# lmxyy/sige

Hardware: AMD Instinct MI355X
Metric: DDPM-256 U-Net sparse (SIGE) forwards/s (higher is better)
Workload: dtype f32; 1 GPU; DDPM 256x256 church U-Net (ch128, mult 1-1-2-2-4-4, 113.7M params, random init), 1.2% square edit, one edited image per GPU, hipGraph replay, NHWC activations, in-place scatter ...; batch_per_gpu=1, resolution=256, parallelism=dp1

## Files before the change

### include/sige_hip.h

```cpp
#ifndef SIGE_HIP_H
#define SIGE_HIP_H

#include <stddef.h>
#include <stdint.h>

#ifdef __cplusplus
extern "C" {
#endif

#define SIGE_HIP_VERSION 310

enum {
    SIGE_HIP_OK = 0,
    SIGE_HIP_EINVAL = -1,
    SIGE_HIP_EUNSUPPORTED = -2,
    SIGE_HIP_ELAUNCH = -3,
    SIGE_HIP_ENODEVICE = -4
};

enum { SIGE_HIP_ACT_IDENTITY = 0, SIGE_HIP_ACT_SWISH = 1,
       SIGE_HIP_ACT_RELU = 2, SIGE_HIP_ACT_LEAKY = 3 , SIGE_HIP_ACT_TANH = 4 };

enum {
    SIGE_HIP_TUNE_CONV_TILE_MT = 0,
// ... 77 lines not shown
                            uint8_t *out, void *stream);
int sige_hip_mask_pyramid_levels(int H, int W, int min_h, int min_w, int *hs, int *ws, int capacity);
int sige_hip_mask_pyramid_u8(const uint8_t *mask, int H, int W, int min_h, int min_w,
                             int dilationH, int dilationW, float threshold, float eps,
                             float *scratch, size_t scratch_floats, uint8_t *out, void *stream);

int sige_hip_reduce_mask_capacity(int H, int W, int strideH, int strideW, int padH, int padW);
int sige_hip_reduce_mask_i32(const uint8_t *mask, int H, int W, int bH, int bW,
                             int strideH, int strideW, int padH, int padW,
                             int32_t *indices, int capacity, int32_t *count, void *stream);

int sige_hip_demand_tiles_capacity(int Hp, int Wp, int tileH, int tileW);
int sige_hip_demand_tiles_i32(const int32_t *indices, const int32_t *count, int capacity, int bH, int bW,
                              int inH, int inW, int upsample2x, int Hp, int Wp, int tileH, int tileW,
                              int padH, int padW, int depth, int32_t *lists, int32_t *counts, void *stream);

size_t sige_hip_block_conv_packed_size(int Cout, int Cin, int kH, int kW, int R, int S,
                                       int strideH, int strideW, int groups);
int sige_hip_block_conv_pack_f32(const float *w, int Cout, int Cin, int kH, int kW,
                                 float *packed, void *stream);
int sige_hip_block_conv_f32(const float *x, int T, int Cin, int R, int S,
                            const float *packed, const float *bias, int Cout, int kH, int kW,
                            int strideH, int strideW, float *out, void *stream);
int sige_hip_block_conv_direct_f32(const float *x, int T, int Cin, int R, int S,
                                   const float *w, const float *bias, int Cout, int kH, int kW,
                                   int strideH, int strideW, int dilationH, int dilationW, int groups,
                                   float *out, void *stream);
int sige_hip_spade_modulate_nhwc_f32(
        const float *x_full, const float *x_tiles, const int32_t *map_x, int Nx, int Rx, int Sx,
        const float *scale, int scaleB, int scaleC, const float *shift, int shiftB, int shiftC,
// ... 287 lines not shown
```

### sige_amd/csrc/mask_pipeline.hip

```cpp
#include "common.hpp"

namespace sige {

constexpr int kMPThreads = 1024;

__global__ void difference_mask_kernel(const float *__restrict__ a, const float *__restrict__ b, int C, long HW,
                                       long strideC, long stridePix, float eps, uint8_t *__restrict__ out) {
    for (long p = (long)blockIdx.x * blockDim.x + threadIdx.x; p < HW; p += (long)gridDim.x * blockDim.x) {
        bool any = false;
        for (int c = 0; c < C; ++c) {
            const long o = c * strideC + p * stridePix;
            any |= fabsf(a[o] - b[o]) > eps;
        }
        out[p] = any ? 1 : 0;
    }
}

__device__ __forceinline__ uint8_t dilated(const uint8_t *__restrict__ m, int W, int h, int w, int dH, int dW, int lo, int hi) {
    if (m[(size_t)h * W + w]) return 1;
    for (int i = 1; i <= dH; ++i) {
        if (h - i >= lo && m[(size_t)(h - i) * W + w]) return 1;
        if (h + i < hi && m[(size_t)(h + i) * W + w]) return 1;
    }
    for (int i = 1; i <= dW; ++i) {
// ... 67 lines not shown
            auto at = [&](int y, int x) -> float {
                const size_t q = (size_t)y * w + x;
                return cur ? cur[q] : (mask[q] ? 1.0f : 0.0f);
            };
            nxt[p] = hy * (hx * at(y0, x0) + lx * at(y0, x1)) + ly * (hx * at(y1, x0) + lx * at(y1, x1));
        }
        __syncthreads();
        cur = nxt;
        nxt = (nxt == level_a) ? level_b : level_a;
        h = h2; w = w2;
    }
}

constexpr int kDTThreads = 1024, kDTMaxPix = 16384, kDTMaxCells = 4096;

__global__ __launch_bounds__(kDTThreads) void demand_tiles_kernel(
        const int32_t *__restrict__ idx, const int32_t *__restrict__ count, int capacity, int bH, int bW, int inH, int inW, int up,
        int Hp, int Wp, int oH, int oW, int padH, int padW, int depth, int32_t *__restrict__ lists, int32_t *__restrict__ counts) {
    __shared__ uint8_t s_map[2][kDTMaxPix];
    __shared__ uint8_t s_flag[kDTMaxCells];
    const int tid = threadIdx.x;
    const int npix = Hp * Wp, gh = (Hp + oH - 1) / oH, gw = (Wp + oW - 1) / oW, ncell = gh * gw;
    for (int p = tid; p < npix; p += kDTThreads) s_map[0][p] = 0;
    __syncthreads();
    int n = *count;
    n = n < 0 ? 0 : (n > capacity ? capacity : n);
    const int bpix = bH * bW;
    for (long i = tid; i < (long)n * bpix; i += kDTThreads) {
        const int t = (int)(i / bpix), r = (int)(i % bpix);
        const int y = idx[2 * t] + r / bW, x = idx[2 * t + 1] + r % bW;
        if (y < 0 || y >= inH || x < 0 || x >= inW) continue;
        const int py = y >> up, px = x >> up;
        if (py < Hp && px < Wp) s_map[0][py * Wp + px] = 1;
    }
    __syncthreads();
    int cur = 0;
    for (int k = 0; k < depth; ++k) {
        const uint8_t *m = s_map[cur];
        for (int c = tid; c < ncell; c += kDTThreads) {
            const int y0 = (c / gw) * oH, x0 = (c % gw) * oW;
            const int y1 = y0 + oH < Hp ? y0 + oH : Hp, x1 = x0 + oW < Wp ? x0 + oW : Wp;
            uint8_t any = 0;
            for (int y = y0; y < y1; ++y)
                for (int x = x0; x < x1; ++x) any |= m[y * Wp + x];
            s_flag[c] = any;
        }
        __syncthreads();
        int32_t *main_list = lists + (size_t)k * ncell * 2, *flat_list = lists + ((size_t)depth + k) * ncell * 2;
        for (int c = tid; c < ncell; c += kDTThreads) {
            if (!s_flag[c] && c != ncell - 1) continue;
            int rank = 0;
            for (int j = 0; j < c; ++j) rank += s_flag[j];
            if (s_flag[c]) {
                const int y0 = (c / gw) * oH, x0 = (c % gw) * oW;
                main_list[2 * rank] = y0 - padH; main_list[2 * rank + 1] = x0 - padW;
                flat_list[2 * rank] = y0; flat_list[2 * rank + 1] = x0;
            }
            if (c == ncell - 1) counts[k] = rank + s_flag[c];
        }
        if (k + 1 < depth) {
            uint8_t *d = s_map[cur ^ 1];
            for (int p = tid; p < npix; p += kDTThreads) {
                const int y = p / Wp, x = p % Wp;
                uint8_t any = 0;
                for (int yy = (y > 0 ? y - 1 : 0); yy <= (y + 1 < Hp ? y + 1 : Hp - 1); ++yy)
                    for (int xx = (x > 0 ? x - 1 : 0); xx <= (x + 1 < Wp ? x + 1 : Wp - 1); ++xx) any |= m[yy * Wp + xx];
                d[p] = any;
            }
        }
        __syncthreads();
        cur ^= 1;
    }
}

}

using namespace sige;

extern "C" int sige_hip_demand_tiles_capacity(int Hp, int Wp, int tileH, int tileW) {
    if (Hp <= 0 || Wp <= 0 || tileH <= 0 || tileW <= 0) return SIGE_HIP_EINVAL;
    return ((Hp + tileH - 1) / tileH) * ((Wp + tileW - 1) / tileW);
}

extern "C" int sige_hip_demand_tiles_i32(const int32_t *indices, const int32_t *count, int capacity, int bH, int bW,
                                         int inH, int inW, int upsample2x, int Hp, int Wp, int tileH, int tileW,
                                         int padH, int padW, int depth, int32_t *lists, int32_t *counts, void *stream) {
    SIGE_PLAN_HOOK(sige_hip_demand_tiles_i32, indices, count, capacity, bH, bW, inH, inW, upsample2x, Hp, Wp, tileH, tileW, padH, padW, depth, lists, counts, stream);
    if (capacity < 0 || bH <= 0 || bW <= 0 || inH <= 0 || inW <= 0 || Hp <= 0 || Wp <= 0 || tileH <= 0 || tileW <= 0 ||
        padH < 0 || padW < 0 || depth <= 0)
        return SIGE_HIP_EINVAL;
    if (!count || !lists || !counts || (capacity > 0 && !indices)) return SIGE_HIP_EINVAL;
    const int up = upsample2x ? 1 : 0;
    if (inH != (Hp << up) || inW != (Wp << up)) return SIGE_HIP_EINVAL;
    if (stacked_shift(Hp) != 0) return SIGE_HIP_EUNSUPPORTED;
    if ((long)Hp * Wp > kDTMaxPix || sige_hip_demand_tiles_capacity(Hp, Wp, tileH, tileW) > kDTMaxCells) return SIGE_HIP_EUNSUPPORTED;
    demand_tiles_kernel<<<1, kDTThreads, 0, as_stream(stream)>>>(indices, count, capacity, bH, bW, inH, inW, up, Hp, Wp, tileH, tileW,
                                                                padH, padW, depth, lists, counts);
    return launch_status();
}

extern "C" int sige_hip_difference_mask_u8(const float *a, const float *b, int C, int H, int W,
                                           int64_t strideC, int64_t strideH, int64_t strideW, float eps,
                                           uint8_t *out, void *stream) {
    SIGE_PLAN_HOOK(sige_hip_difference_mask_u8, a, b, C, H, W, strideC, strideH, strideW, eps, out, stream);
    if (C <= 0 || H <= 0 || W <= 0) return SIGE_HIP_EINVAL;
    if (!a || !b || !out) return SIGE_HIP_EINVAL;
    if (strideH != (int64_t)W * strideW) return SIGE_HIP_EUNSUPPORTED;
    const long HW = (long)H * W;
    const int blocks = (int)((HW + 255) / 256 < 2048 ? (HW + 255) / 256 : 2048);
    difference_mask_kernel<<<blocks, 256, 0, as_stream(stream)>>>(a, b, C, HW, strideC, strideW, eps, out);
    return launch_status();
}
// ... 48 lines not shown
```

### sige_amd/hip.py

```python
import ctypes
import os
import threading
from typing import Optional, Tuple

import torch

_PKG = os.path.dirname(os.path.abspath(__file__))
LIB_PATH = os.environ.get("SIGE_HIP_LIB", os.path.join(_PKG, "lib", "libsige_hip.so"))

ACT = {"identity": 0, "swish": 1}
ACT_EXT = {"identity": 0, "relu": 2, "leaky": 3, "tanh": 4}

_c_int, _c_vp, _c_sz = ctypes.c_int, ctypes.c_void_p, ctypes.c_size_t
_lib = None

_BC = [_c_vp, _c_int, _c_int, _c_int, _c_int]

_SIGNATURES = {
    "sige_hip_version": (_c_int, []),
    "sige_hip_error_string": (ctypes.c_char_p, [_c_int]),
    "sige_hip_device_arch": (ctypes.c_char_p, []),
    "sige_hip_launch_count": (ctypes.c_int64, []),
    "sige_hip_last_launch_device": (_c_int, []),
    "sige_hip_preload": (_c_int, []),
# ... 4 lines not shown
    "sige_hip_tile_table_i32": (_c_int, [_c_vp] + [_c_int] * 9 + [_c_vp, _c_vp]),
    "sige_hip_scatter_fused_f32": (_c_int, [_c_vp, _c_vp] + [_c_int] * 6 + [_c_vp, _c_int, _c_int, _c_int] + _BC + [_c_vp, _c_vp]),
    "sige_hip_scatter_with_block_residual_fused_f32": (
        _c_int, [_c_vp] * 4 + [_c_int] * 8 + [_c_vp, _c_int, _c_int, _c_int] * 2 + [_c_vp, _c_vp]),
    "sige_hip_scatter_map_i32": (_c_int, [_c_int] * 10 + [_c_vp, _c_int, _c_vp, _c_vp]),
    "sige_hip_scatter_gather_f32": (
        _c_int, [_c_vp, _c_vp] + [_c_int] * 8 + [_c_vp, _c_int, _c_vp] + _BC + _BC + [_c_int, _c_int, _c_vp, _c_vp]),
    "sige_hip_difference_mask_u8": (_c_int, [_c_vp, _c_vp] + [_c_int] * 3 + [ctypes.c_int64] * 3 + [ctypes.c_float, _c_vp, _c_vp]),
    "sige_hip_dilate_mask_u8": (_c_int, [_c_vp] + [_c_int] * 4 + [_c_vp, _c_vp]),
    "sige_hip_mask_pyramid_levels": (_c_int, [_c_int] * 4 + [_c_vp, _c_vp, _c_int]),
    "sige_hip_mask_pyramid_u8": (_c_int, [_c_vp] + [_c_int] * 6 + [ctypes.c_float] * 2 + [_c_vp, _c_sz, _c_vp, _c_vp]),
    "sige_hip_reduce_mask_capacity": (_c_int, [_c_int] * 6),
    "sige_hip_reduce_mask_i32": (_c_int, [_c_vp] + [_c_int] * 8 + [_c_vp, _c_int, _c_vp, _c_vp]),
    "sige_hip_demand_tiles_capacity": (_c_int, [_c_int] * 4),
    "sige_hip_demand_tiles_i32": (_c_int, [_c_vp, _c_vp] + [_c_int] * 13 + [_c_vp, _c_vp, _c_vp]),
    "sige_hip_block_conv_packed_size": (_c_sz, [_c_int] * 9),
    "sige_hip_block_conv_packed_size_f16c": (_c_sz, [_c_int] * 9),
    "sige_hip_block_conv_pack_f16c": (_c_int, [_c_vp] + [_c_int] * 4 + [_c_vp, _c_vp]),
    "sige_hip_block_conv_pack_f32": (_c_int, [_c_vp] + [_c_int] * 4 + [_c_vp, _c_vp]),
    "sige_hip_block_conv_f32": (_c_int, [_c_vp] + [_c_int] * 4 + [_c_vp, _c_vp] + [_c_int] * 5 + [_c_vp, _c_vp]),
    "sige_hip_gather_conv_f32": (
        _c_int, [_c_vp] + [_c_int] * 6 + [_c_vp, _c_int] + _BC + _BC + [_c_int, _c_vp, _c_vp] + [_c_int] * 5 + [_c_vp, _c_vp]),
    "sige_hip_scatter_gather_conv_f32": (
        _c_int, [_c_vp, _c_vp] + [_c_int] * 8 + [_c_vp, _c_int, _c_vp] + _BC + _BC + [_c_int, _c_vp, _c_vp]
        + [_c_int] * 5 + [_c_vp, _c_vp]),
    "sige_hip_gather_conv_nchw_f32": (
        _c_int, [_c_vp, _c_vp] + [_c_int] * 7 + [_c_vp, _c_int] + [_c_vp, _c_int, _c_int] * 2 + [_c_int, _c_vp, _c_vp]
        + [_c_int] * 7 + [_c_vp, _c_int, _c_int, _c_vp, _c_vp]),
    "sige_hip_group_norm_affine_workspace": (_c_sz, [_c_int] * 5),
    "sige_hip_group_norm_affine_f32": (_c_int, [_c_vp] + [_c_int] * 5 + [ctypes.c_float] + [_c_vp] * 6),
# ... 505 lines not shown
                                          _stream(m)), "reduce_mask")
    n = int(count[0].item())
    return buf[:n].clone()


class DemandTiles:

    def __init__(self, main, flat, cells: int):
        self.main, self.flat, self.cells = list(main), list(flat), int(cells)

    @property
    def counts(self):
        return [int(t.shape[0]) for t in self.main]


def reduce_mask_batch(requests, demands=None):
    if not requests:
        return [] if demands is None else ([], [])
    dev = requests[0][0].device
    n_req = len(requests)
    counts = torch.empty(n_req + sum(d[6] for d in demands or ()), dtype=torch.int32, device=dev)
    bufs = []
    for i, (mask, block, stride, padding) in enumerate(requests):
        if mask.dim() != 2 or not mask.is_cuda or mask.device != dev:
            raise RuntimeError("sige_amd.hip.reduce_mask_batch: expected 2-D masks on one GPU")
        m = mask if mask.dtype in (torch.bool, torch.uint8) else (mask != 0)
        m = m.contiguous()
        H, W = m.shape
        cap = lib().sige_hip_reduce_mask_capacity(H, W, stride[0], stride[1], padding[0], padding[1])
        buf = torch.empty((max(cap, 1), 2), dtype=torch.int32, device=dev)
        _check(lib().sige_hip_reduce_mask_i32(m.data_ptr(), H, W, block[0], block[1], stride[0], stride[1],
                                              padding[0], padding[1], buf.data_ptr(), cap,
                                              counts.data_ptr() + 4 * i, _stream(m)), "reduce_mask")
        bufs.append((buf, m, cap))
    dbufs, at = [], n_req
    for (i, in_res, up, prod_res, out_tile, pad, depth) in demands or ():
        buf, m, cap = bufs[i]
        block = requests[i][1]
        cells = lib().sige_hip_demand_tiles_capacity(prod_res[0], prod_res[1], out_tile[0], out_tile[1])
        if cells <= 0:
            raise RuntimeError("sige_amd.hip.reduce_mask_batch: bad demand-region geometry")
        lists = torch.empty((2, depth, cells, 2), dtype=torch.int32, device=dev)
        _check(lib().sige_hip_demand_tiles_i32(buf.data_ptr(), counts.data_ptr() + 4 * i, cap, block[0], block[1], in_res[0], in_res[1],
                                               int(bool(up)), prod_res[0], prod_res[1], out_tile[0], out_tile[1], pad[0], pad[1],
                                               depth, lists.data_ptr(), counts.data_ptr() + 4 * at, _stream(m)), "demand_tiles")
        dbufs.append((lists, at, depth, cells))
        at += depth
    rec = plan_recorder()
    if rec is not None:
        first = rec.new_slots(counts.numel())
        _check(lib().sige_hip_plan_record_readback(rec.handle, counts.data_ptr(), first, counts.numel()), "plan_record_readback")
        ns = counts.cpu().tolist()
        out = []
        for i, ((buf, m, _), n) in enumerate(zip(bufs, ns)):
            rec.bind_index_list(buf, first + i, n)
            rec.keep.extend((buf, m))
            out.append(buf[:n])
        dout = []
        for lists, at, depth, cells in dbufs:
            for g in range(2):
                for k in range(depth):
                    rec.bind_index_list(lists[g, k], first + at + k, ns[at + k])
            rec.keep.append(lists)
            dout.append(DemandTiles([lists[0, k, :ns[at + k]] for k in range(depth)],
                                    [lists[1, k, :ns[at + k]] for k in range(depth)], cells))
        rec.keep.append(counts)
        return out if demands is None else (out, dout)
    ns = counts.cpu().tolist()
    out = [buf[:n].clone() for (buf, _, _), n in zip(bufs, ns)]
    if demands is None:
        return out
    dout = [DemandTiles([lists[0, k, :ns[at + k]] for k in range(depth)], [lists[1, k, :ns[at + k]] for k in range(depth)], cells)
            for lists, at, depth, cells in dbufs]
    return out, dout


def difference_mask(tensor1: torch.Tensor, tensor2: torch.Tensor, eps: float) -> torch.Tensor:
    if tensor1.shape != tensor2.shape:
        raise RuntimeError("difference_mask: shapes differ")
    a, b = tensor1, tensor2
    if a.dim() == 4:
        assert a.shape[0] == 1
        a, b = a[0], b[0]
    if a.dim() == 2:
        a, b = a[None], b[None]
    if a.dim() != 3:
        raise NotImplementedError("Unknown mask dimension [%d]!!!" % tensor1.dim())
    if not (a.is_cuda and b.is_cuda and a.dtype == b.dtype == torch.float32):
        raise NotImplementedError("difference_mask: fp32 GPU tensors")
# ... 1358 lines not shown
```

### sige_amd/nn/base.py

```python
from typing import Dict, List, Optional, Tuple

import torch
from torch import nn
from torch.nn import functional as F

from .. import runtime as _runtime
from . import deferred

MODES = ("full", "sparse", "profile")


class _RuntimeTable(dict):

    def __init__(self, function_name: str):
        super().__init__()
        self.function_name = function_name

    def __missing__(self, device_type: str):
        fn = _runtime.resolve(device_type, self.function_name)
        if fn is not None:
            self[device_type] = fn
        return fn


# ... 198 lines not shown
        for m in self._sige_modules():
            if isinstance(m, Gather) and m.input_res is not None and not m.verbose:
                res = tuple(m.input_res)
                mask = masks.get(res)
                key = m.index_key(res)
                if mask is not None and mask.is_cuda and mask.dim() == 2 and key not in cache and key not in keys:
                    keys.append(key)
                    reqs.append((mask, m.block_size, m.block_stride, m.offset))
        self._demand_lists = {}
        demands = []
        for name, g, up, prod_res, depth in self._demand_requests(masks):
            key = g.index_key(tuple(g.input_res))
            if key in keys:
                demands.append((name, ("demand_tiles", *key[1:], int(up), *prod_res, *g.out_tile, *g.offset, depth),
                                (keys.index(key), tuple(g.input_res), up, tuple(prod_res), tuple(g.out_tile), tuple(g.offset), depth)))
        if reqs:
            from .. import hip

            lists, regions = hip.reduce_mask_batch(reqs, [d[2] for d in demands])
            for key, idx in zip(keys, lists):
                cache[key] = idx
            for (name, key, _), region in zip(demands, regions):
                cache[key] = region
                self._demand_lists[name] = region

    def _demand_requests(self, masks):
        return []

    def adopt_index_lists(self, view_of):
        for region in getattr(self, "_demand_lists", {}).values():
            for lists in (region.main, region.flat):
                for k, t in enumerate(lists):
                    v = view_of(t)
                    if v is not None:
                        lists[k] = v

    def set_mode(self, mode: str):
        self.mode = mode
        for module in self._sige_modules():
            module.set_mode(mode)

    def clear_cache(self):
        for module in self._sige_modules():
            module.clear_cache()

# ... 48 lines not shown
```

### sige_amd/nn/dense.py

```python
from typing import Optional, Tuple

import torch
from torch import nn
from torch.nn import functional as F

_GEOMETRY = {
    ((3, 3), (1, 1), (1, 1)): ((6, 6), (4, 4), (1, 1)),
    ((1, 1), (1, 1), (0, 0)): ((4, 4), (4, 4), (0, 0)),
    ((3, 3), (2, 2), (0, 0)): ((5, 5), (2, 2), (0, 0)),
}


def _tile_compute(compute: str) -> str:
    return compute if compute in ("f16", "f16x3") else "f32"


WIDE_MIN_FLOP = {3: 4.0e9, 1: 2.0e9}
WIDE_MIN_FLOP_X3 = {3: 4.0e9, 1: 2.0e9}
WIDE_MIN_FLOP_FULL_PASS = {3: 0.25e9, 1: 2.0e9}
WIDE_MIN_FLOP_F32 = {3: 1.0e30, 1: 1.0e30}
WIDE_MIN_FLOP_F32_STACKED = {3: 8.0e9, 1: 1.0e30}
FULL_PASS_F32_NATIVE = False
TILE_X3_MIN_FLOP = 2.0e9

# ... 144 lines not shown
            made = scatter.emulated_twins(out, twins)
    out._sige_twins = made
    return out


def demand_buffer(conv: nn.Conv2d, name, shape, device) -> torch.Tensor:
    bufs = conv.__dict__.setdefault("_sige_demand_bufs", {})
    buf = bufs.get(name)
    if buf is None or tuple(buf.shape) != tuple(shape) or buf.device != device:
        buf = torch.zeros(tuple(shape), dtype=torch.float32, device=device).contiguous(memory_format=torch.channels_last)
        bufs[name] = buf
    return buf


def _demand_twin_buffers(conv: nn.Conv2d, keys, shape, device):
    bufs = conv.__dict__.setdefault("_sige_demand_bufs", {})
    for name in [n for n in bufs if isinstance(n, tuple) and n[0] == "twin" and n[1] not in keys]:
        del bufs[name]
    return [demand_buffer(conv, ("twin", k), shape, device) for k in keys]


def _fused_conv2d(conv, x, scale, shift, activation_name, x2, residual, pad_bottom_right, out_affine, twins=None, made=None,
                  tiles=None, out_buf=None):
    if x.is_cuda and x.dtype == torch.float32 and fusable(conv):
        from .. import hip

        block, out_tile, offset = _GEOMETRY[(tuple(conv.kernel_size), tuple(conv.stride), tuple(conv.padding))]
        partial = (tiles is not None and out_buf is not None and not pad_bottom_right and conv.stride[0] == 1 and hip.is_cl(x)
                   and (x2 is None or (hip.is_cl(x2) and hip.cat_fusable(x.shape[0], x.shape[1], conv.kernel_size)))
                   and hip.cl_supported(x.shape[1], 0 if x2 is None else x2.shape[1], conv.out_channels))
        if partial:
            B, _, H, W = x.shape
# ... 120 lines not shown
```

### sige_amd/plan.py

```python
import ctypes
from typing import Callable, Dict, Optional

import torch

from . import hip
from .graphs import GraphPool
from .nn.base import SIGEModel
from .nn.gather import Gather

MASKS, FORWARD = 0, 1


class _Recorder:

    def __init__(self, plan: "LaunchPlan", section: int):
        self.plan = plan
        self.handle = plan.handle
        self.section = section
        self.keep = plan._keep
        self.idx_info = plan._idx_info

    def new_slots(self, n: int) -> int:
        first = hip.lib().sige_hip_plan_new_slots(self.handle, n)
        if first < 0:
# ... 67 lines not shown
            raise ValueError("LaunchPlan.record: `mask` must be a 2-D bool tensor on the GPU")
        self.build_masks, self.forward = build_masks, forward
        with torch.cuda.device(self.device):
            self.mask = mask.clone()
            self.model.set_mode("sparse")
            self.model.set_masks(build_masks(self.mask))
            eager = None
            for _ in range(max(1, warmup)):
                eager = forward()
            eager = eager.clone()
            with LaunchPlan._Recording(self, MASKS):
                self.model.set_masks(build_masks(self.mask))
                for m in self._scatter_modules():
                    m.plan_tables()
                    m.refresh_outputs(new_mask=True)
            torch.cuda.synchronize(self.device)
            self.pool = GraphPool(self.device)
            with LaunchPlan._Recording(self, FORWARD):
                self._record_graph, self.out = self.pool.capture(forward)
            if hip.lib().sige_hip_plan_calls(self.handle, FORWARD) <= 0:
                raise RuntimeError("LaunchPlan.record: the forward made no library call")
            self._read_counts()
            self._recorded_counts = list(self.counts)
            if not all(self.counts):
                raise RuntimeError("LaunchPlan.record: record under a mask with at least one active tile at every resolution (an empty "
                                   "index list hands the entry points a null pointer, which no later mask can be looked up under)")
            out = self.run()
            if check:
                torch.cuda.synchronize(self.device)
                err = float((out - eager).abs().max())
# ... 83 lines not shown
```

### sige_amd/utils.py

```python
from typing import Dict, Optional, Tuple, Union

import numpy as np
import torch
from torch.nn import functional as F

IntPair = Union[int, Tuple[int, int]]


def _pair(v: IntPair) -> Tuple[int, int]:
    return (v, v) if isinstance(v, int) else (int(v[0]), int(v[1]))


def reduce_mask(
    mask: torch.Tensor,
    block_size: Optional[IntPair],
    stride: Optional[IntPair],
    padding: Optional[IntPair],
    verbose: bool = False,
) -> Optional[torch.Tensor]:
    if block_size is None or stride is None or padding is None:
        return None
    block_size, stride, padding = _pair(block_size), _pair(stride), _pair(padding)
    if mask.is_cuda:
        from . import hip
# ... 121 lines not shown
    for k in range(depth):
        padded = torch.zeros((gh * oh, gw * ow), dtype=torch.bool)
        padded[:hp, :wp] = need
        cells = torch.nonzero(padded.reshape(gh, oh, gw, ow).any(dim=3).any(dim=1))
        origin = torch.stack((cells[:, 0] * oh, cells[:, 1] * ow), dim=1).to(torch.int32)
        flat.append(origin.contiguous())
        main.append((origin - torch.tensor([ph, pw], dtype=torch.int32)).contiguous())
        if k + 1 < depth:
            grown = need.clone()
            for dy in (-1, 0, 1):
                for dx in (-1, 0, 1):
                    src = need[max(-dy, 0):hp - max(dy, 0), max(-dx, 0):wp - max(dx, 0)]
                    grown[max(dy, 0):hp - max(-dy, 0), max(dx, 0):wp - max(-dx, 0)] |= src
            need = grown
    return main, flat
```

### sige_amd/workloads/ddpm_unet.py

```python
import math
from dataclasses import dataclass
from typing import Optional, Tuple

import torch
from torch import nn
from torch.nn import functional as F

from ..nn import Gather, Scatter, ScatterGather, ScatterWithBlockResidual, SIGEConv2d, SIGEModel, SIGEModule, paired_convs
from ..nn.deferred import lazy_cat
from ..nn.dense import demand_buffer, fast_full_pass, full_conv2d, fused_conv2d, group_norm_affine, input_conv2d


@dataclass
class DDPMConfig:
    ch: int = 128
    ch_mult: Tuple[int, ...] = (1, 1, 2, 2, 4, 4)
    num_res_blocks: int = 2
    attn_resolutions: Tuple[int, ...] = (16,)
    in_ch: int = 3
    out_ch: int = 3
    resolution: int = 256
    main_block: Optional[int] = 6
    shortcut_block: Optional[int] = 4
    sparse_threshold: int = 64
# ... 207 lines not shown

    def _pairing(self, t: torch.Tensor):
        return paired_convs(t, enabled=self.pair and self.cin != self.cout and self.mode == "sparse")

    def forward(self, x, temb: Optional[torch.Tensor], demand=None) -> torch.Tensor:
        pair = x if isinstance(x, (tuple, list)) else None
        if self.mode == "full":
            if pair and not self.plain and self._fast_full() and pair[0].is_cuda:
                return self._full(pair[0], temb, x2=pair[1])
            return self._full(torch.cat(pair, dim=1) if pair else x, temb)
        if self.mode in ("sparse", "profile"):
            if pair and not self.sparse_main and self.mode == "sparse":
                return self._sparse_dense(pair[0], pair[1], demand)
            if pair and self.mode == "sparse" and self.cin != self.cout:
                return self._sparse(lazy_cat(pair[0], pair[1]))
            return self._sparse(torch.cat(pair, dim=1) if pair else x)
        raise NotImplementedError("Unknown mode [%s]!!!" % self.mode)

    def _fast_full(self) -> bool:
        from ..nn import dense as _dense

        return _dense.fast_full_pass(self.conv1)

    def _shortcut(self, x, x2=None):
        if self.cin == self.cout:
            return x if x2 is None else torch.cat([x, x2], dim=1)
        if x2 is not None:
            if self.sparse_shortcut:
                self.shortcut_gather.note_full_input(x.shape[2:])
            return full_conv2d(self.nin_shortcut, x, x2=x2)
        if self.sparse_shortcut:
# ... 28 lines not shown
            s2, t2 = norm_affine(h + _as4(te), self.norm2, fast)
            t2 = t2 + te * s2
        self._drop_twin_links()
        self.affine[self.cache_id] = tuple(_as4(v).contiguous() for v in (s1, t1, s2, t2))
        if self.sparse_main and self.preactivate:
            self.scatter_gather.cache_activated(_as4(s2), _as4(t2))
        if self.sparse_main and self.sparse_shortcut:
            if fast and h.is_cuda:
                h = full_conv2d(self.conv2, h, _as4(s2), _as4(t2), "swish", residual=skip, stats=True)
                return self.scatter(h, skip, x_is_sum=True)
            h = full_conv2d(self.conv2, h, _as4(s2), _as4(t2), "swish")
            return self.scatter(h, skip)
        h = full_conv2d(self.conv2, h, _as4(s2), _as4(t2), "swish", residual=skip, stats=fast)
        return self.scatter(h) if self.sparse_main else h

    def _sparse(self, x):
        s1, t1, s2, t2 = self.affine[self.cache_id]
        if self.sparse_main and self.preactivate and self.mode == "sparse":
            parts = list(x.parts) if hasattr(x, "parts") else [x]
            first = parts[0]
            tw = self._twin_inputs(parts, s1, t1)
            with self._pairing(first):
                skip, join = (self._shortcut_async(lambda: self._shortcut(x), first) if self.cin != self.cout
                              else (x, lambda: None))
                if tw is not None:
                    xa = tw[0] if len(tw) == 1 else lazy_cat(tw[0], tw[1])
                    h = self.conv1(self.main_gather(xa, preactivated=True), out_affine=(s2, t2, "swish"))
                else:
                    h = self.conv1(self.main_gather(x, s1, t1), out_affine=(s2, t2, "swish"))
            tiles = self.scatter_gather(h, preactivated=True)
            join()
            return self._produced(self.scatter.forward_fused(self.conv2, tiles, skip))
        if not self.sparse_main:
            return self._sparse_dense(x, None)
        skip = self._shortcut(x)
        h = self.conv1(self.main_gather(x, s1, t1))
        if self.mode == "sparse":
            return self.scatter.forward_fused(self.conv2, self.scatter_gather(h, s2, t2), skip)
        return self.scatter(self.conv2(self.scatter_gather(h, s2, t2)), skip)

    def _demand_args(self, conv, demand, deeper: int, x) -> dict:
        if demand is None:
            return {}
        from .. import hip

        region, depth = demand
        lists = region.flat if tuple(conv.kernel_size) == (1, 1) else region.main
        tiles = lists[depth + deeper]
        if tiles.shape[0] == region.cells and hip.plan_recorder() is None:
            return {}
        shape = (x.shape[0], conv.out_channels, x.shape[2], x.shape[3])
        return dict(tiles=tiles, out=demand_buffer(conv, "out", shape, x.device))

    def _sparse_dense(self, x, x2, demand=None):
        s1, t1, s2, t2 = self.affine[self.cache_id]
        join = lambda: None
        if self.preactivate:
            tw = self._twin_inputs([x] if x2 is None else [x, x2], s1, t1)
            with self._pairing(x):
                if self.cin == self.cout:
                    skip = x if x2 is None else torch.cat([x, x2], dim=1)
                else:
                    skip, join = self._shortcut_async(lambda: fused_conv2d(self.nin_shortcut, x, x2=x2,
                                                                           **self._demand_args(self.nin_shortcut, demand, 0, x)), x)
                if tw is not None:
                    h = fused_conv2d(self.conv1, tw[0], None, None, "identity", x2=(tw[1] if len(tw) > 1 else None),
                                     out_affine=(s2, t2, "swish"), **self._demand_args(self.conv1, demand, 1, x))
# ... 394 lines not shown
        if not (self.DENSE_ON_DEMAND and self.mode == "sparse" and self.edit_batch == 1 and isinstance(h, torch.Tensor) and h.is_cuda):
            return None
        region = getattr(self, "_demand_lists", {}).get("up.%d" % lvl)
        if region is None or h.shape[0] != 1:
            return None
        from .. import hip

        convs = [c for b in stage.block for c in (b.conv1, b.conv2, getattr(b, "nin_shortcut", None)) if c is not None]
        if not hip.is_cl(h) or any(getattr(c, "compute_dtype", "f32") != "f32" for c in convs):
            return None
        g = stage.upsample.gather
        if not g.fuses_upsample(h) or tuple(g.input_res) != (2 * h.shape[2], 2 * h.shape[3]):
            return None
        return region

    def forward(self, x: torch.Tensor, t: torch.Tensor) -> torch.Tensor:
        assert x.shape[2] == x.shape[3] == self.resolution
        temb = self._temb(t)
        nxt = (lambda: temb.pop(0)) if temb is not None else (lambda: None)

        from ..nn import dense as _dense

        native_full = self.mode == "full" and x.is_cuda and not getattr(self.conv_in, "_plain_model", False) and (
            getattr(self.conv_out, "compute_dtype", "f32") != "f32" or _dense.FULL_PASS_F32_NATIVE)
        h0 = self._conv_in(x, native_full)
        if x.is_contiguous(memory_format=torch.channels_last) and not x.is_contiguous():
            h0 = h0.contiguous(memory_format=torch.channels_last)
        E = self.edit_batch
        if E > 1:
            if self.mode != "sparse" or x.shape[0] != E:
                raise RuntimeError("stacked edits: sparse mode, one input image per edit")
            from ..stacked import tall, untall

            h0 = tall(h0)
        hs = [h0]
        for lvl, stage in enumerate(self.down):
            for i, block in enumerate(stage.block):
                h = block(hs[-1], nxt())
                if len(stage.attn):
                    h = stage.attn[i](h)
                hs.append(h)
            if lvl != self.num_levels - 1:
                hs.append(stage.downsample(hs[-1]))

        h = self.mid.block_1(hs[-1], nxt())
        h = self.mid.attn_1(h)
        h = self.mid.block_2(h, nxt())

        for lvl in reversed(range(self.num_levels)):
            stage = self.up[lvl]
            region = self._stage_demand(lvl, stage, h)
            for i, block in enumerate(stage.block):
                if region is not None:
# ... 15 lines not shown
```

Before: 817.8 forward/s.

## Restrict dense down-stage convs to change regions grown from the sparse mask

Adds a change-tiles kernel that projects the downsample's active blocks to the next level and dilates them once per 3x3 conv, producing per-conv tile lists of cells whose output can differ from the cached original. Dense down stages without attention then run their convs only on those tiles, writing into persistent tagged output buffers. The buffers are first filled by a full-tile build pass keyed by a signature. This cuts work at dense down levels but adds state tracking, a cache-invalidation signature and an extra tile-list kernel, and it is only correct while the cached buffers stay valid.

```diff
diff --git a/include/sige_hip.h b/include/sige_hip.h
--- a/include/sige_hip.h
+++ b/include/sige_hip.h
@@ -115,6 +115,11 @@
 int sige_hip_demand_tiles_i32(const int32_t *indices, const int32_t *count, int capacity, int bH, int bW,
                               int inH, int inW, int upsample2x, int Hp, int Wp, int tileH, int tileW,
                               int padH, int padW, int depth, int32_t *lists, int32_t *counts, void *stream);
+
+int sige_hip_change_tiles_i32(const int32_t *indices, const int32_t *count, int capacity, int bH, int bW,
+                              int strideH, int strideW, int offsetH, int offsetW, int outH, int outW,
+                              int Hp, int Wp, int tileH, int tileW, int padH, int padW, int depth,
+                              int32_t *lists, int32_t *counts, void *stream);
 
 size_t sige_hip_block_conv_packed_size(int Cout, int Cin, int kH, int kW, int R, int S,
                                        int strideH, int strideW, int groups);
diff --git a/sige_amd/csrc/mask_pipeline.hip b/sige_amd/csrc/mask_pipeline.hip
--- a/sige_amd/csrc/mask_pipeline.hip
+++ b/sige_amd/csrc/mask_pipeline.hip
@@ -105,13 +105,51 @@
 
 constexpr int kDTThreads = 1024, kDTMaxPix = 16384, kDTMaxCells = 4096;
 
+__device__ __forceinline__ void dt_compact(const uint8_t *m, uint8_t *s_flag, int Hp, int Wp, int oH, int oW, int padH, int padW,
+                                           int32_t *__restrict__ main_list, int32_t *__restrict__ flat_list, int32_t *__restrict__ n_out) {
+    const int tid = threadIdx.x;
+    const int gh = (Hp + oH - 1) / oH, gw = (Wp + oW - 1) / oW, ncell = gh * gw;
+    for (int c = tid; c < ncell; c += kDTThreads) {
+        const int y0 = (c / gw) * oH, x0 = (c % gw) * oW;
+        const int y1 = y0 + oH < Hp ? y0 + oH : Hp, x1 = x0 + oW < Wp ? x0 + oW : Wp;
+        uint8_t any = 0;
+        for (int y = y0; y < y1; ++y)
+            for (int x = x0; x < x1; ++x) any |= m[y * Wp + x];
+        s_flag[c] = any;
+    }
+    __syncthreads();
+    for (int c = tid; c < ncell; c += kDTThreads) {
+        if (!s_flag[c] && c != ncell - 1) continue;
+        int rank = 0;
+        for (int j = 0; j < c; ++j) rank += s_flag[j];
+        if (s_flag[c]) {
+            const int y0 = (c / gw) * oH, x0 = (c % gw) * oW;
+            main_list[2 * rank] = y0 - padH; main_list[2 * rank + 1] = x0 - padW;
+            flat_list[2 * rank] = y0; flat_list[2 * rank + 1] = x0;
+        }
+        if (c == ncell - 1) *n_out = rank + s_flag[c];
+    }
+    __syncthreads();
+}
+
+__device__ __forceinline__ void dt_dilate(const uint8_t *m, uint8_t *d, int Hp, int Wp) {
+    for (int p = threadIdx.x; p < Hp * Wp; p += kDTThreads) {
+        const int y = p / Wp, x = p % Wp;
+        uint8_t any = 0;
+        for (int yy = (y > 0 ? y - 1 : 0); yy <= (y + 1 < Hp ? y + 1 : Hp - 1); ++yy)
+            for (int xx = (x > 0 ? x - 1 : 0); xx <= (x + 1 < Wp ? x + 1 : Wp - 1); ++xx) any |= m[yy * Wp + xx];
+        d[p] = any;
+    }
+    __syncthreads();
+}
+
 __global__ __launch_bounds__(kDTThreads) void demand_tiles_kernel(
         const int32_t *__restrict__ idx, const int32_t *__restrict__ count, int capacity, int bH, int bW, int inH, int inW, int up,
         int Hp, int Wp, int oH, int oW, int padH, int padW, int depth, int32_t *__restrict__ lists, int32_t *__restrict__ counts) {
     __shared__ uint8_t s_map[2][kDTMaxPix];
     __shared__ uint8_t s_flag[kDTMaxCells];
     const int tid = threadIdx.x;
-    const int npix = Hp * Wp, gh = (Hp + oH - 1) / oH, gw = (Wp + oW - 1) / oW, ncell = gh * gw;
+    const int npix = Hp * Wp, ncell = ((Hp + oH - 1) / oH) * ((Wp + oW - 1) / oW);
     for (int p = tid; p < npix; p += kDTThreads) s_map[0][p] = 0;
     __syncthreads();
     int n = *count;
@@ -127,40 +165,40 @@
     __syncthreads();
     int cur = 0;
     for (int k = 0; k < depth; ++k) {
-        const uint8_t *m = s_map[cur];
-        for (int c = tid; c < ncell; c += kDTThreads) {
-            const int y0 = (c / gw) * oH, x0 = (c % gw) * oW;
-            const int y1 = y0 + oH < Hp ? y0 + oH : Hp, x1 = x0 + oW < Wp ? x0 + oW : Wp;
-            uint8_t any = 0;
-            for (int y = y0; y < y1; ++y)
-                for (int x = x0; x < x1; ++x) any |= m[y * Wp + x];
-            s_flag[c] = any;
-        }
-        __syncthreads();
-        int32_t *main_list = lists + (size_t)k * ncell * 2, *flat_list = lists + ((size_t)depth + k) * ncell * 2;
-        for (int c = tid; c < ncell; c += kDTThreads) {
-            if (!s_flag[c] && c != ncell - 1) continue;
-            int rank = 0;
-            for (int j = 0; j < c; ++j) rank += s_flag[j];
-            if (s_flag[c]) {
-                const int y0 = (c / gw) * oH, x0 = (c % gw) * oW;
-                main_list[2 * rank] = y0 - padH; main_list[2 * rank + 1] = x0 - padW;
-                flat_list[2 * rank] = y0; flat_list[2 * rank + 1] = x0;
-            }
-            if (c == ncell - 1) counts[k] = rank + s_flag[c];
-        }
-        if (k + 1 < depth) {
-            uint8_t *d = s_map[cur ^ 1];
-            for (int p = tid; p < npix; p += kDTThreads) {
-                const int y = p / Wp, x = p % Wp;
-                uint8_t any = 0;
-                for (int yy = (y > 0 ? y - 1 : 0); yy <= (y + 1 < Hp ? y + 1 : Hp - 1); ++yy)
-                    for (int xx = (x > 0 ? x - 1 : 0); xx <= (x + 1 < Wp ? x + 1 : Wp - 1); ++xx) any |= m[yy * Wp + xx];
-                d[p] = any;
-            }
-        }
-        __syncthreads();
+        dt_compact(s_map[cur], s_flag, Hp, Wp, oH, oW, padH, padW, lists + (size_t)k * ncell * 2,
+                   lists + ((size_t)depth + k) * ncell * 2, counts + k);
+        if (k + 1 < depth) dt_dilate(s_map[cur], s_map[cur ^ 1], Hp, Wp);
         cur ^= 1;
+    }
+}
+
+__global__ __launch_bounds__(kDTThreads) void change_tiles_kernel(
+        const int32_t *__restrict__ idx, const int32_t *__restrict__ count, int capacity, int sH, int sW, int offH, int offW,
+        int tH, int tW, int Hp, int Wp, int oH, int oW, int padH, int padW, int depth, int32_t *__restrict__ lists,
+        int32_t *__restrict__ counts) {
+    __shared__ uint8_t s_map[2][kDTMaxPix];
+    __shared__ uint8_t s_flag[kDTMaxCells];
+    const int tid = threadIdx.x;
+    const int npix = Hp * Wp, ncell = ((Hp + oH - 1) / oH) * ((Wp + oW - 1) / oW);
+    for (int p = tid; p < npix; p += kDTThreads) s_map[0][p] = 0;
+    __syncthreads();
+    int n = *count;
+    n = n < 0 ? 0 : (n > capacity ? capacity : n);
+    const int tpix = tH * tW;
+    for (long i = tid; i < (long)n * tpix; i += kDTThreads) {
+        const int t = (int)(i / tpix), r = (int)(i % tpix);
+        const int ty = idx[2 * t] + offH, tx = idx[2 * t + 1] + offW;
+        if (ty < 0 || tx < 0) continue;
+        const int y = ty / sH + r / tW, x = tx / sW + r % tW;
+        if (y < Hp && x < Wp) s_map[0][y * Wp + x] = 1;
+    }
+    __syncthreads();
+    int cur = 0;
+    for (int k = 0; k < depth; ++k) {
+        dt_dilate(s_map[cur], s_map[cur ^ 1], Hp, Wp);
+        cur ^= 1;
+        dt_compact(s_map[cur], s_flag, Hp, Wp, oH, oW, padH, padW, lists + (size_t)k * ncell * 2,
+                   lists + ((size_t)depth + k) * ncell * 2, counts + k);
     }
 }
 
@@ -187,6 +225,23 @@
     if ((long)Hp * Wp > kDTMaxPix || sige_hip_demand_tiles_capacity(Hp, Wp, tileH, tileW) > kDTMaxCells) return SIGE_HIP_EUNSUPPORTED;
     demand_tiles_kernel<<<1, kDTThreads, 0, as_stream(stream)>>>(indices, count, capacity, bH, bW, inH, inW, up, Hp, Wp, tileH, tileW,
                                                                 padH, padW, depth, lists, counts);
+    return launch_status();
+}
+
+extern "C" int sige_hip_change_tiles_i32(const int32_t *indices, const int32_t *count, int capacity, int bH, int bW,
+                                         int strideH, int strideW, int offsetH, int offsetW, int outH, int outW,
+                                         int Hp, int Wp, int tileH, int tileW, int padH, int padW, int depth,
+                                         int32_t *lists, int32_t *counts, void *stream) {
+    SIGE_PLAN_HOOK(sige_hip_change_tiles_i32, indices, count, capacity, bH, bW, strideH, strideW, offsetH, offsetW, outH, outW, Hp, Wp, tileH, tileW, padH, padW, depth, lists, counts, stream);
+    if (capacity < 0 || bH <= 0 || bW <= 0 || strideH <= 0 || strideW <= 0 || offsetH < 0 || offsetW < 0 || outH <= 0 || outW <= 0 ||
+        Hp <= 0 || Wp <= 0 || tileH <= 0 || tileW <= 0 || padH < 0 || padW < 0 || depth <= 0)
+        return SIGE_HIP_EINVAL;
+    if (!count || !lists || !counts || (capacity > 0 && !indices)) return SIGE_HIP_EINVAL;
+    if ((long)(outH - 1) * strideH >= bH || (long)(outW - 1) * strideW >= bW) return SIGE_HIP_EINVAL;
+    if (stacked_shift(Hp) != 0) return SIGE_HIP_EUNSUPPORTED;
+    if ((long)Hp * Wp > kDTMaxPix || sige_hip_demand_tiles_capacity(Hp, Wp, tileH, tileW) > kDTMaxCells) return SIGE_HIP_EUNSUPPORTED;
+    change_tiles_kernel<<<1, kDTThreads, 0, as_stream(stream)>>>(indices, count, capacity, strideH, strideW, offsetH, offsetW, outH, outW,
+                                                                Hp, Wp, tileH, tileW, padH, padW, depth, lists, counts);
     return launch_status();
 }
 
diff --git a/sige_amd/hip.py b/sige_amd/hip.py
--- a/sige_amd/hip.py
+++ b/sige_amd/hip.py
@@ -42,6 +42,7 @@
     "sige_hip_reduce_mask_i32": (_c_int, [_c_vp] + [_c_int] * 8 + [_c_vp, _c_int, _c_vp, _c_vp]),
     "sige_hip_demand_tiles_capacity": (_c_int, [_c_int] * 4),
     "sige_hip_demand_tiles_i32": (_c_int, [_c_vp, _c_vp] + [_c_int] * 13 + [_c_vp, _c_vp, _c_vp]),
+    "sige_hip_change_tiles_i32": (_c_int, [_c_vp, _c_vp] + [_c_int] * 16 + [_c_vp, _c_vp, _c_vp]),
     "sige_hip_block_conv_packed_size": (_c_sz, [_c_int] * 9),
     "sige_hip_block_conv_packed_size_f16c": (_c_sz, [_c_int] * 9),
     "sige_hip_block_conv_pack_f16c": (_c_int, [_c_vp] + [_c_int] * 4 + [_c_vp, _c_vp]),
@@ -577,12 +578,17 @@
         return [int(t.shape[0]) for t in self.main]
 
 
-def reduce_mask_batch(requests, demands=None):
+class ChangeTiles(DemandTiles):
+    """Index lists of a dense stage's change regions (include/sige_hip.h: sige_hip_change_tiles_i32): `main[k-1]` / `flat[k-1]` =
+    the cells on which the output of the stage's k-th 3x3 conv can differ from the original's, in the 3x3 and the 1x1 geometry."""
+
+
+def reduce_mask_batch(requests, demands=None, changes=None):
     if not requests:
-        return [] if demands is None else ([], [])
+        return [] if demands is None else (([], []) if changes is None else ([], [], []))
     dev = requests[0][0].device
     n_req = len(requests)
-    counts = torch.empty(n_req + sum(d[6] for d in demands or ()), dtype=torch.int32, device=dev)
+    counts = torch.empty(n_req + sum(d[6] for d in demands or ()) + sum(c[7] for c in changes or ()), dtype=torch.int32, device=dev)
     bufs = []
     for i, (mask, block, stride, padding) in enumerate(requests):
         if mask.dim() != 2 or not mask.is_cuda or mask.device != dev:
@@ -607,7 +613,21 @@
         _check(lib().sige_hip_demand_tiles_i32(buf.data_ptr(), counts.data_ptr() + 4 * i, cap, block[0], block[1], in_res[0], in_res[1],
                                                int(bool(up)), prod_res[0], prod_res[1], out_tile[0], out_tile[1], pad[0], pad[1],
                                                depth, lists.data_ptr(), counts.data_ptr() + 4 * at, _stream(m)), "demand_tiles")
-        dbufs.append((lists, at, depth, cells))
+        dbufs.append((lists, at, depth, cells, DemandTiles))
+        at += depth
+    n_dem = len(dbufs)
+    for (i, stride, wrote, offset, prod_res, out_tile, pad, depth) in changes or ():
+        buf, m, cap = bufs[i]
+        block = requests[i][1]
+        cells = lib().sige_hip_demand_tiles_capacity(prod_res[0], prod_res[1], out_tile[0], out_tile[1])
+        if cells <= 0:
+            raise RuntimeError("sige_amd.hip.reduce_mask_batch: bad change-region geometry")
+        lists = torch.empty((2, depth, cells, 2), dtype=torch.int32, device=dev)
+        _check(lib().sige_hip_change_tiles_i32(buf.data_ptr(), counts.data_ptr() + 4 * i, cap, block[0], block[1], stride[0], stride[1],
+                                               offset[0], offset[1], wrote[0], wrote[1], prod_res[0], prod_res[1],
+                                               out_tile[0], out_tile[1], pad[0], pad[1], depth, lists.data_ptr(),
+                                               counts.data_ptr() + 4 * at, _stream(m)), "change_tiles")
+        dbufs.append((lists, at, depth, cells, ChangeTiles))
         at += depth
     rec = plan_recorder()
     if rec is not None:
@@ -620,22 +640,22 @@
             rec.keep.extend((buf, m))
             out.append(buf[:n])
         dout = []
-        for lists, at, depth, cells in dbufs:
+        for lists, at, depth, cells, kind in dbufs:
             for g in range(2):
                 for k in range(depth):
                     rec.bind_index_list(lists[g, k], first + at + k, ns[at + k])
             rec.keep.append(lists)
-            dout.append(DemandTiles([lists[0, k, :ns[at + k]] for k in range(depth)],
-                                    [lists[1, k, :ns[at + k]] for k in range(depth)], cells))
+            dout.append(kind([lists[0, k, :ns[at + k]] for k in range(depth)],
+                             [lists[1, k, :ns[at + k]] for k in range(depth)], cells))
         rec.keep.append(counts)
-        return out if demands is None else (out, dout)
-    ns = counts.cpu().tolist()
-    out = [buf[:n].clone() for (buf, _, _), n in zip(bufs, ns)]
-    if demands is None:
-        return out
-    dout = [DemandTiles([lists[0, k, :ns[at + k]] for k in range(depth)], [lists[1, k, :ns[at + k]] for k in range(depth)], cells)
-            for lists, at, depth, cells in dbufs]
-    return out, dout
+    else:
+        ns = counts.cpu().tolist()
+        out = [buf[:n].clone() for (buf, _, _), n in zip(bufs, ns)]
+        dout = [kind([lists[0, k, :ns[at + k]] for k in range(depth)], [lists[1, k, :ns[at + k]] for k in range(depth)], cells)
+                for lists, at, depth, cells, kind in dbufs]
+    if changes is not None:
+        return out, dout[:n_dem], dout[n_dem:]
+    return out if demands is None else (out, dout)
 
 
 def difference_mask(tensor1: torch.Tensor, tensor2: torch.Tensor, eps: float) -> torch.Tensor:
diff --git a/sige_amd/nn/base.py b/sige_amd/nn/base.py
--- a/sige_amd/nn/base.py
+++ b/sige_amd/nn/base.py
@@ -236,21 +236,34 @@
             if key in keys:
                 demands.append((name, ("demand_tiles", *key[1:], int(up), *prod_res, *g.out_tile, *g.offset, depth),
                                 (keys.index(key), tuple(g.input_res), up, tuple(prod_res), tuple(g.out_tile), tuple(g.offset), depth)))
+        self._change_lists = {}
+        changes = []
+        for name, g, prod_res, depth in self._change_requests(masks):
+            key = g.index_key(tuple(g.input_res))
+            if key in keys:
+                changes.append((name, ("change_tiles", *key[1:], *g.model_stride, *g.out_tile, *prod_res, depth),
+                                (keys.index(key), tuple(g.model_stride), tuple(g.out_tile), tuple(g.offset), tuple(prod_res), (4, 4), (1, 1), depth)))
         if reqs:
             from .. import hip
 
-            lists, regions = hip.reduce_mask_batch(reqs, [d[2] for d in demands])
+            lists, regions, cregions = hip.reduce_mask_batch(reqs, [d[2] for d in demands], [c[2] for c in changes])
             for key, idx in zip(keys, lists):
                 cache[key] = idx
             for (name, key, _), region in zip(demands, regions):
                 cache[key] = region
                 self._demand_lists[name] = region
+            for (name, key, _), region in zip(changes, cregions):
+                cache[key] = region
+                self._change_lists[name] = region
 
     def _demand_requests(self, masks):
         return []
 
+    def _change_requests(self, masks):
+        return []
+
     def adopt_index_lists(self, view_of):
-        for region in getattr(self, "_demand_lists", {}).values():
+        for region in list(getattr(self, "_demand_lists", {}).values()) + list(getattr(self, "_change_lists", {}).values()):
             for lists in (region.main, region.flat):
                 for k, t in enumerate(lists):
                     v = view_of(t)
diff --git a/sige_amd/nn/dense.py b/sige_amd/nn/dense.py
--- a/sige_amd/nn/dense.py
+++ b/sige_amd/nn/dense.py
@@ -182,8 +182,12 @@
 
 
 def _demand_twin_buffers(conv: nn.Conv2d, keys, shape, device):
+    from .scatter import twin_key_cache_id
+
     bufs = conv.__dict__.setdefault("_sige_demand_bufs", {})
-    for name in [n for n in bufs if isinstance(n, tuple) and n[0] == "twin" and n[1] not in keys]:
+    cids = {twin_key_cache_id(k) for k in keys}
+    for name in [n for n in bufs if isinstance(n, tuple) and n[0] == "twin" and n[1] not in keys
+                 and (twin_key_cache_id(n[1]) is None or twin_key_cache_id(n[1]) in cids)]:
         del bufs[name]
     return [demand_buffer(conv, ("twin", k), shape, device) for k in keys]
 
diff --git a/sige_amd/plan.py b/sige_amd/plan.py
--- a/sige_amd/plan.py
+++ b/sige_amd/plan.py
@@ -105,6 +105,9 @@
                 for m in self._scatter_modules():
                     m.plan_tables()
                     m.refresh_outputs(new_mask=True)
+                refresh = getattr(self.model, "refresh_change_stages", None)
+                if refresh is not None:
+                    refresh()
             torch.cuda.synchronize(self.device)
             self.pool = GraphPool(self.device)
             with LaunchPlan._Recording(self, FORWARD):
diff --git a/sige_amd/utils.py b/sige_amd/utils.py
--- a/sige_amd/utils.py
+++ b/sige_amd/utils.py
@@ -159,3 +159,45 @@
                     grown[max(dy, 0):hp - max(-dy, 0), max(dx, 0):wp - max(-dx, 0)] |= src
             need = grown
     return main, flat
+
+
+def change_tiles(
+    active_indices: torch.Tensor,
+    block_size: IntPair,
+    stride: IntPair,
+    offset: IntPair,
+    written_tile: IntPair,
+    stage_res: IntPair,
+    out_tile: IntPair = 4,
+    padding: IntPair = 1,
+    depth: int = 1,
+):
+    (bh, bw), (sh, sw), (fh, fw) = _pair(block_size), _pair(stride), _pair(offset)
+    (th, tw), (hp, wp) = _pair(written_tile), _pair(stage_res)
+    (oh, ow), (ph, pw) = _pair(out_tile), _pair(padding)
+    if min(bh, bw, sh, sw, th, tw, hp, wp, oh, ow, depth) <= 0 or min(fh, fw, ph, pw) < 0:
+        raise ValueError("change_tiles: sizes must be positive, offsets and paddings non-negative")
+    if (th - 1) * sh >= bh or (tw - 1) * sw >= bw:
+        raise ValueError("change_tiles: the written tile does not fit the block at this stride")
+    changed = torch.zeros((hp, wp), dtype=torch.bool)
+    for y0, x0 in active_indices.cpu().tolist():
+        if y0 + fh < 0 or x0 + fw < 0:
+            continue
+        y, x = (y0 + fh) // sh, (x0 + fw) // sw
+        changed[y:y + th, x:x + tw] = True
+    gh, gw = -(-hp // oh), -(-wp // ow)
+    main, flat = [], []
+    for _ in range(depth):
+        grown = changed.clone()
+        for dy in (-1, 0, 1):
+            for dx in (-1, 0, 1):
+                src = changed[max(-dy, 0):hp - max(dy, 0), max(-dx, 0):wp - max(dx, 0)]
+                grown[max(dy, 0):hp - max(-dy, 0), max(dx, 0):wp - max(-dx, 0)] |= src
+        changed = grown
+        padded = torch.zeros((gh * oh, gw * ow), dtype=torch.bool)
+        padded[:hp, :wp] = changed
+        cells = torch.nonzero(padded.reshape(gh, oh, gw, ow).any(dim=3).any(dim=1))
+        origin = torch.stack((cells[:, 0] * oh, cells[:, 1] * ow), dim=1).to(torch.int32)
+        flat.append(origin.contiguous())
+        main.append((origin - torch.tensor([ph, pw], dtype=torch.int32)).contiguous())
+    return main, flat
diff --git a/sige_amd/workloads/ddpm_unet.py b/sige_amd/workloads/ddpm_unet.py
--- a/sige_amd/workloads/ddpm_unet.py
+++ b/sige_amd/workloads/ddpm_unet.py
@@ -245,7 +245,7 @@
                 return self._sparse_dense(pair[0], pair[1], demand)
             if pair and self.mode == "sparse" and self.cin != self.cout:
                 return self._sparse(lazy_cat(pair[0], pair[1]))
-            return self._sparse(torch.cat(pair, dim=1) if pair else x)
+            return self._sparse(torch.cat(pair, dim=1) if pair else x, demand)
         raise NotImplementedError("Unknown mode [%s]!!!" % self.mode)
 
     def _fast_full(self) -> bool:
@@ -304,7 +304,7 @@
         h = full_conv2d(self.conv2, h, _as4(s2), _as4(t2), "swish", residual=skip, stats=fast)
         return self.scatter(h) if self.sparse_main else h
 
-    def _sparse(self, x):
+    def _sparse(self, x, demand=None):
         s1, t1, s2, t2 = self.affine[self.cache_id]
         if self.sparse_main and self.preactivate and self.mode == "sparse":
             parts = list(x.parts) if hasattr(x, "parts") else [x]
@@ -322,7 +322,7 @@
             join()
             return self._produced(self.scatter.forward_fused(self.conv2, tiles, skip))
         if not self.sparse_main:
-            return self._sparse_dense(x, None)
+            return self._sparse_dense(x, None, demand)
         skip = self._shortcut(x)
         h = self.conv1(self.main_gather(x, s1, t1))
         if self.mode == "sparse":
@@ -337,10 +337,11 @@
         region, depth = demand
         lists = region.flat if tuple(conv.kernel_size) == (1, 1) else region.main
         tiles = lists[depth + deeper]
-        if tiles.shape[0] == region.cells and hip.plan_recorder() is None:
+        tag, keep = getattr(region, "tag", None), getattr(region, "keep", False)
+        if tiles.shape[0] == region.cells and hip.plan_recorder() is None and not keep:
             return {}
         shape = (x.shape[0], conv.out_channels, x.shape[2], x.shape[3])
-        return dict(tiles=tiles, out=demand_buffer(conv, "out", shape, x.device))
+        return dict(tiles=tiles, out=demand_buffer(conv, "out" if tag is None else ("out", tag), shape, x.device))
 
     def _sparse_dense(self, x, x2, demand=None):
         s1, t1, s2, t2 = self.affine[self.cache_id]
@@ -765,6 +766,140 @@
             return None
         return region
 
+    DENSE_ON_CHANGE = True
+
+    def _change_stages(self):
+        out = []
+        for lvl in range(1, len(self.down)):
+            stage, prev = self.down[lvl], getattr(self.down[lvl - 1], "downsample", None)
+            if prev is None or not prev.sparse or len(stage.attn) or prev.gather.input_res is None:
+                continue
+            if any(b.sparse_main or not b.preactivate or b.overlap for b in stage.block):
+                continue
+            if min(prev.gather.input_res) // 2 <= 4 * len(stage.block):
+                continue
+            out.append((lvl, stage, prev))
+        return out
+
+    def _change_requests(self, masks):
+        if not self.DENSE_ON_CHANGE or self.edit_batch != 1:
+            return []
+        reqs = []
+        for lvl, stage, prev in self._change_stages():
+            g = prev.gather
+            res = tuple(g.input_res)
+            mask = masks.get(res)
+            if mask is None or not mask.is_cuda or mask.dim() != 2 or res[0] % 2 or res[1] % 2 or tuple(g.model_stride) != (2, 2):
+                continue
+            reqs.append(("down.%d" % lvl, g, (res[0] // 2, res[1] // 2), 2 * len(stage.block)))
+        if reqs:
+            from .. import hip
+
+            if hip.get_edit_batch() != 1:
+                return []
+        return reqs
+
+    def _change_signature(self, lvl: int, stage, h):
+        cid = stage.block[0].cache_id
+        sct = self.down[lvl - 1].downsample.scatter
+        blocks = tuple((b._aff_gen, tuple(v.data_ptr() for v in b.affine[cid]), tuple(b._my_twins())) for b in stage.block)
+        return (self.timestamp, h.data_ptr(), tuple(h.shape), str(h.device), sct._out_bufs.gen.get(cid, 0), blocks)
+
+    @staticmethod
+    def _change_buffers(stage, cid):
+        from ..nn.scatter import twin_key_cache_id
+
+        out = []
+        for b in stage.block:
+            for conv in (b.conv1, b.conv2, getattr(b, "nin_shortcut", None)):
+                for name, buf in (conv.__dict__.get("_sige_demand_bufs", {}) if conv is not None else {}).items():
+                    if name == ("out", cid) or (isinstance(name, tuple) and name[0] == "twin" and twin_key_cache_id(name[1]) == cid):
+                        out.append((id(conv), repr(name), buf.data_ptr()))
+        return tuple(out)
+
+    def _stage_change(self, lvl: int, stage, h, refresh: bool = False):
+        if not (self.DENSE_ON_CHANGE and self.mode == "sparse" and self.edit_batch == 1 and isinstance(h, torch.Tensor) and h.is_cuda):
+            return None
+        region = getattr(self, "_change_lists", {}).get("down.%d" % lvl)
+        if region is None or h.shape[0] != 1 or len(region.main) != 2 * len(stage.block):
+            return None
+        from .. import hip
+
+        convs = [c for b in stage.block for c in (b.conv1, b.conv2, getattr(b, "nin_shortcut", None)) if c is not None]
+        if not hip.is_cl(h) or h.dtype != torch.float32 or any(getattr(c, "compute_dtype", "f32") != "f32" for c in convs):
+            return None
+        if any(b.sparse_update or b.mode != "sparse" for b in stage.block):
+            return None
+        g = self.down[lvl - 1].downsample.gather
+        if tuple(g.input_res) != (2 * h.shape[2], 2 * h.shape[3]) or region.cells != -(-h.shape[2] // 4) * -(-h.shape[3] // 4):
+            return None
+        cid = stage.block[0].cache_id
+        self.__dict__.setdefault("_change_inputs", {})[(lvl, cid)] = h
+        planned = hip.plan_recorder() is not None
+        counts = region.counts
+        if not planned and not refresh and (counts[0] == 0 or counts[0] == region.cells):
+            return None
+        sig = self._change_signature(lvl, stage, h)
+        state = self.__dict__.setdefault("_change_state", {})
+        if refresh or state.get((lvl, cid)) != (sig, self._change_buffers(stage, cid)):
+            every = (hip.all_tiles(h.shape[2], h.shape[3], (4, 4), (1, 1), (1, 1), h.device),
+                     hip.all_tiles(h.shape[2], h.shape[3], (4, 4), (1, 1), (0, 0), h.device))
+            per_block = []
+            for _ in stage.block:
+                r = hip.DemandTiles([every[0]] * 2, [every[1]] * 2, region.cells)
+                r.tag, r.keep = cid, True
+                per_block.append(r)
+            state.pop((lvl, cid), None)
+            return per_block, ((lvl, cid), sig)
+        return self._change_steady(stage, region, cid), None
+
+    @staticmethod
+    def _change_steady(stage, region, cid):
+        from .. import hip
+
+        per_block = []
+        for i in range(len(stage.block)):
+            r = hip.DemandTiles([region.main[2 * i + 1], region.main[2 * i]], [region.flat[2 * i + 1], region.flat[2 * i]], region.cells)
+            r.tag, r.keep = cid, False
+            per_block.append(r)
+        return per_block
+
+    def refresh_change_stages(self):
+        inputs = self.__dict__.get("_change_inputs", {})
+        state = self.__dict__.setdefault("_change_state", {})
+        for (lvl, cid), h in list(inputs.items()):
+            stage = self.down[lvl]
+            state.pop((lvl, cid), None)
+            if stage.block[0].cache_id != cid or cid not in stage.block[0].affine:
+                continue
+            found = self._stage_change(lvl, stage, h, refresh=True)
+            if found is None:
+                continue
+            per_block, (key, sig) = found
+            with torch.no_grad():
+                built = self._change_build(lvl, stage, h, per_block, sig)
+            if built is not None:
+                state[key] = (built, self._change_buffers(stage, cid))
+
+    def _change_build(self, lvl: int, stage, h, per_block, sig):
+        for _ in range(3):
+            x = h
+            for i, block in enumerate(stage.block):
+                x = block(x, None, demand=(per_block[i], 0))
+            after = self._change_signature(lvl, stage, h)
+            if after == sig:
+                return sig
+            sig = after
+        return None
+
+    def rebuild_derived_caches(self):
+        self.refresh_change_stages()
+
+    def clear_cache(self):
+        super().clear_cache()
+        self.__dict__.pop("_change_inputs", None)
+        self.__dict__.pop("_change_state", None)
+
     def forward(self, x: torch.Tensor, t: torch.Tensor) -> torch.Tensor:
         assert x.shape[2] == x.shape[3] == self.resolution
         temb = self._temb(t)
@@ -786,8 +921,16 @@
             h0 = tall(h0)
         hs = [h0]
         for lvl, stage in enumerate(self.down):
+            change = self._stage_change(lvl, stage, hs[-1]) if lvl else None
+            if change is not None and change[0][0].keep:
+                key, sig = change[1]
+                built = self._change_build(lvl, stage, hs[-1], change[0], sig)
+                if built is not None:
+                    if not torch.cuda.is_current_stream_capturing():
+                        self._change_state[key] = (built, self._change_buffers(stage, key[1]))
+                    change = (self._change_steady(stage, self._change_lists["down.%d" % lvl], key[1]), None)
             for i, block in enumerate(stage.block):
-                h = block(hs[-1], nxt())
+                h = block(hs[-1], nxt()) if change is None else block(hs[-1], nxt(), demand=(change[0][i], 0))
                 if len(stage.attn):
                     h = stage.attn[i](h)
                 hs.append(h)
```

New measurement: 834.3 forward/s (median of 6 runs). 2.0% higher.
